# zraorg/ZRA

Measured on AMD Instinct MI355X. Metric: compress + RA-decompress GiB/s, 16 GiB @ 64 KiB frames, 1/2/4/8 MI355X, higher is better.
Workload: dtype u8

## Files before the change

### zra_amd/csrc/zra_encode.hip

```cpp
#include <cstdio>
#include <unistd.h>
#include "zra_host.h"
#include "zra_dev.h"
#include "zra_format.h"
#include "zra_env.h"
#include <algorithm>
#include <cstdlib>
#include <vector>

extern "C" __global__ void zra_mf_kernel(ZraEncArgs a, uint32_t block, uint32_t only, uint32_t onlySlot, uint32_t perWave);
extern "C" __global__ void zra_mf_opt_kernel(ZraEncArgs a, uint32_t block, uint32_t only, uint32_t onlySlot, uint32_t perWave);
extern "C" __global__ void zra_mf_dfast_ls_kernel(ZraEncArgs a, uint32_t block, uint32_t only, uint32_t onlySlot);
extern "C" __global__ void zra_mf_hc_kernel(ZraEncArgs a, uint32_t block, uint32_t only, uint32_t onlySlot);
extern "C" __global__ void zra_mf_fast_kernel(ZraEncArgs a, uint32_t block, uint32_t perWave);
extern "C" __global__ void zra_mf_dfast_kernel(ZraEncArgs a, uint32_t block, uint32_t only, uint32_t onlySlot);
extern "C" __global__ void zra_mf_dfast_fl_kernel(ZraEncArgs a, ZraFlagArgs g, uint32_t block, uint32_t only, uint32_t onlySlot);
extern "C" __global__ void zra_entropy_kernel(ZraEncArgs a, uint32_t block);
extern "C" __global__ void zra_entropy_front_kernel(ZraEncArgs a, uint32_t block);
extern "C" __global__ void zra_entropy_back_kernel(ZraEncArgs a, uint32_t block);
extern "C" __global__ void zra_ent_chain_kernel(ZraEncArgs a);
extern "C" __global__ void zra_ent_chain5_kernel(ZraEncArgs a);

using namespace zra_dev;
using namespace zra_env;
// ... 186 lines not shown
  HIPCHK(hipMemsetAsync(encScan_.p, 0, 64 + 4 * nEntLaunches, stream2_));
  size_t entLaunch = 0;

  ZraEncArgs base{};
  base.in = dIn; base.inSize = inSize; base.frameSize = frameSize; base.checksum = checksum ? 1 : 0;
  base.full = full; base.tail = tail;
  dbgSeqStride_ = seqStride; dbgB_ = (uint32_t)B;
  base.tableStride = tableWords; base.seqStride = seqStride; base.litStride = litStride; base.slotStride = slotStride;
  base.entWorkStride = entWorkStride; base.slotRing = B; base.entSubFrames = B; base.entPrio = 3;

  size_t evNext = 0;
  auto ev = [&]() -> hipEvent_t {
    if (evNext == evPool_.size()) { hipEvent_t e = nullptr; if (hipEventCreate(&e) != hipSuccess) return nullptr; evPool_.push_back(e); }
    return evPool_[evNext++];
  };
  std::vector<std::pair<hipEvent_t, hipEvent_t>> mfSpans, entSpans;
  hipEvent_t entDone[2] = {nullptr, nullptr};
  hipStream_t mfStream2 = nullptr;
  if (nCtx == 2) {
    if (!pipeStreams_[0] && hipStreamCreateWithFlags(&pipeStreams_[0], hipStreamNonBlocking) != hipSuccess) { pipeStreams_[0] = nullptr; (void)hipGetLastError(); }
    mfStream2 = pipeStreams_[0];
  }
  { hipEvent_t e0 = ev(); if (!e0) return zerr(1); HIPCHK(hipEventRecord(e0, stream_)); HIPCHK(hipStreamWaitEvent(stream2_, e0, 0));
    if (mfStream2) HIPCHK(hipStreamWaitEvent(mfStream2, e0, 0)); }

  uint64_t batchIdx = 0;
  for (uint64_t f0 = 0; f0 < nFramesTotal; f0 += B, batchIdx++) {
    const uint32_t nb = (uint32_t)std::min<uint64_t>(B, nFramesTotal - f0);
    const int c = (int)(batchIdx % nCtx);
    EncCtx& x = encCtx_[c];
    ZraEncArgs a = base;
    a.firstFrame = (uint32_t)f0; a.nFrames = nb;
    a.tables = x.tables.as<uint32_t>(); a.seqs = x.seqs.as<uint64_t>(); a.lits = x.lits.as<uint8_t>(); a.slots = x.slots.as<uint8_t>();
    a.state = x.misc.as<ZraEncFrameState>();
    a.blockOut = (ZraEncBlockOut*)(x.misc.as<uint8_t>() + (size_t)B * sizeof(ZraEncFrameState));
    a.contentCk = x.ck.as<uint32_t>();
    a.sizes = x.sizes.as<uint64_t>();
    uint64_t* dOffsets = x.sizes.as<uint64_t>() + B;
    if (checksum)
      hipLaunchKernelGGL(zra_content_ck_kernel, dim3((nb * 4 + 255) / 256), dim3(256), 0, stream2_, dIn, (u64)inSize, frameSize, (u32)f0, nb, a.contentCk);
    const uint64_t firstFrameSize = std::min<uint64_t>(frameSize, inSize - f0 * frameSize);
    const ZraEncParams& P0 = firstFrameSize == frameSize ? full : tail;
    const uint32_t rounds = (uint32_t)((firstFrameSize + P0.blockSize - 1) / P0.blockSize);
    hipStream_t sA = (c == 1 && mfStream2) ? mfStream2 : stream_;
    if (entDone[c]) HIPCHK(hipStreamWaitEvent(sA, entDone[c], 0));
    { static const bool poison = env_set("ZRA_ENC_POISON");
      if (poison) HIPCHK(hipMemsetAsync(x.tables.p, 0xA5, (size_t)nb * tableWords * 4, sA)); }
    for (uint32_t blk = 0; blk < rounds; blk++) {
      hipEvent_t m0 = ev(), m1 = ev(), e1 = ev();
      if (!m0 || !m1 || !e1) return zerr(1);
      HIPCHK(hipEventRecord(m0, sA));
      {
        const bool hasTail = tailSize && f0 + nb == nFramesTotal;
        const uint32_t shL = 1, shS = 2, dupLog = 8;
        a.mfFilter = shL | (shS << 4) | (dupLog << 8);
        const uint32_t hl = std::max(full.hashLog, tail.hashLog), cl = std::max(full.chainLog, tail.chainLog);
        const size_t filterBytes = (8u << dupLog) + (((size_t)1 << hl) >> shL) / 8 + (((size_t)1 << cl) >> shS) / 8 + 64;
        const bool serialAll = std::min<uint64_t>(frameSize, inSize) > (1ull << full.windowLog);
        a.serialAll = serialAll ? 1u : 0u;
        const bool oddTail = !serialAll && hasTail && (tail.strategy == 2) != (full.strategy == 2);
        auto launchLone = [&](uint32_t only, uint32_t slot) {
          if (tail.strategy >= 3 && tail.strategy <= 5) hipLaunchKernelGGL(zra_mf_hc_kernel, dim3(1), dim3(64), 0, sA, a, blk, only, slot);
          else hipLaunchKernelGGL(mfGeneric, dim3(1), dim3(64), 0, sA, a, blk, only, slot, 1u);
        };
        if (full.strategy == 2 && !serialAll) {
          hipLaunchKernelGGL(zra_mf_dfast_kernel, dim3(nb), dim3(64), filterBytes, sA, a, blk, 0xFFFFFFFFu, 0u);
          if (oddTail) launchLone((uint32_t)(nb - 1), (uint32_t)(nb - 1));
        } else {
          const bool hashChain = full.strategy >= 3 && full.strategy <= 5 && !serialAll;
          const uint32_t perWave = hashChain ? 1u : std::min<uint32_t>(8u, std::max<uint32_t>(1u, (nb + (uint32_t)numCUs_ * 32 - 1) / ((uint32_t)numCUs_ * 32)));
          const bool lean = hashChain || full.strategy == 1;
          const uint32_t hcPad = hashChain && full.searchLog >= 5 && tableWords * 4 >= (4ull << 20) ? 5120u : 0u;
          if (hashChain) hipLaunchKernelGGL(zra_mf_hc_kernel, dim3(nb), dim3(64), hcPad, sA, a, blk, 0xFFFFFFFFu, 0u);
          else if (lean) hipLaunchKernelGGL(zra_mf_fast_kernel, dim3((nb + perWave - 1) / perWave), dim3(64), 0, sA, a, blk, perWave);
          else hipLaunchKernelGGL(mfGeneric, dim3((nb + perWave - 1) / perWave), dim3(64), 0, sA, a, blk, 0xFFFFFFFFu, 0u, perWave);
          if (oddTail) hipLaunchKernelGGL(zra_mf_dfast_kernel, dim3(1), dim3(64), filterBytes, sA, a, blk, (uint32_t)(nb - 1), (uint32_t)(nb - 1));
          else if (lean && hasTail && (hashChain ? (tail.strategy < 3 || tail.strategy > 5) : tail.strategy != 1))
            launchLone((uint32_t)(nb - 1), (uint32_t)(nb - 1));
        }
      }
      HIPCHK(hipEventRecord(m1, sA));
      mfSpans.push_back({m0, m1});
      HIPCHK(hipStreamWaitEvent(stream2_, m1, 0));
      hipEvent_t e0 = ev(); if (!e0) return zerr(1);
      HIPCHK(hipEventRecord(e0, stream2_));
      { ZraEncArgs ae = a; ae.entQueue = dEntQueues + entLaunch++; ae.entWork = x.work.as<uint8_t>();
        hipLaunchKernelGGL(zra_entropy_kernel, dim3(std::min<uint32_t>(nb, entGridB)), dim3(256), 0, stream2_, ae, blk); }
      HIPCHK(hipEventRecord(e1, stream2_));
      entSpans.push_back({e0, e1});
      if (blk + 1 < rounds) HIPCHK(hipStreamWaitEvent(sA, e1, 0));
    }
    hipLaunchKernelGGL(zra_scan_sizes_kernel, dim3(1), dim3(64), 0, stream2_, a.sizes, nb, dOffsets, dRunning, (const u32*)nullptr);
    hipLaunchKernelGGL(zra_gather_frames_kernel, dim3(nb), dim3(256), 0, stream2_, a.slots, slotStride, a.sizes, dOffsets, dBody,
                       bodyBase0, dEntries ? dEntries : nullptr, (u32)f0, dSizes, (const u32*)nullptr);
    hipEvent_t done = ev(); if (!done) return zerr(1);
    HIPCHK(hipEventRecord(done, stream2_));
    entDone[c] = done;
    if ((uint64_t)env_i64("ZRA_ENC_FAIL_BATCH", -1) == batchIdx) return zerr(1);
  }
  uint64_t total = 0;
  HIPCHK(hipMemcpyAsync(&total, dRunning, 8, hipMemcpyDeviceToHost, stream2_));
  HIPCHK(hipStreamSynchronize(stream2_));
  HIPCHK(hipStreamSynchronize(stream_));
  if (mfStream2) HIPCHK(hipStreamSynchronize(mfStream2));
  HIPCHK(hipGetLastError());
  double kernelMs = 0;
  kstats_[0] = kstats_[1] = kstats_[2] = kstats_[3] = 0;
  for (auto& sp : mfSpans) { float m = 0; if (hipEventElapsedTime(&m, sp.first, sp.second) == hipSuccess) { kstats_[0] += m; kstats_[1] += 1; kernelMs += m; } }
  for (auto& sp : entSpans) { float m = 0; if (hipEventElapsedTime(&m, sp.first, sp.second) == hipSuccess) { kstats_[2] += m; kstats_[3] += 1; } }
  lastKernelMs_ = kernelMs;
// ... 15 lines not shown
  {
    size_t freeB = 0, totalB = 0;
    if (hipMemGetInfo(&freeB, &totalB) != hipSuccess) freeB = 24ull << 30;
    uint64_t mine = 0; for (auto& x : encCtx_) mine += x.seqs.cap;
    budget = std::min<uint64_t>(64ull << 30, std::max<uint64_t>(8ull << 30, ((uint64_t)freeB + mine) / 3));
  }
  uint64_t SBIG = 0, nSuper = 0, subsPerSuper = 0; int nCtx = 1;
  EncCtx& sh = encCtx_[0];
  static const uint32_t entPerCU = (uint32_t)std::max(1, env_int("ZRA_ENT_WGS", 8));
  const uint32_t entGrid = (uint32_t)std::min<uint64_t>((uint64_t)numCUs_ * entPerCU, nFramesTotal);
  const uint64_t entWorkStride = (9 * seqStride + 255) & ~255ull;
  static const int splitEnv = env_int("ZRA_ENT_SPLIT", 1);
  const bool entSplit = splitEnv >= 2 || (splitEnv == 1 && nFramesTotal >= 256);
  uint64_t slotRing = 0;
  for (;; budget /= 2) {
    SBIG = std::max<uint64_t>(1, std::min<uint64_t>(nFramesTotal, budget / perFrame));
    if (SBIG > SB) SBIG -= SBIG % SB;
    nCtx = nFramesTotal > SBIG ? 2 : 1;
    nSuper = (nFramesTotal + SBIG - 1) / SBIG;
    subsPerSuper = (SBIG + SB - 1) / SB;
    slotRing = std::min<uint64_t>(SB, SBIG);
    const uint64_t workUnits = entSplit ? std::min<uint64_t>(SB, nFramesTotal) : entGrid;
    bool okR = sh.tables.reserve((size_t)nSlots * tableWords * 4) && sh.lits.reserve((size_t)entGrid * litStride) && sh.work.reserve((size_t)workUnits * entWorkStride) &&
               sh.slots.reserve(slotRing * slotStride) && (!entSplit || sh.rec.reserve((size_t)workUnits * sizeof(ZraEntRec)));
    for (int c = 0; c < nCtx && okR; c++) {
      EncCtx& x = encCtx_[c];
      okR = x.seqs.reserve(SBIG * seqStride * 8) && x.misc.reserve(SBIG * (sizeof(ZraEncFrameState) + sizeof(ZraEncBlockOut))) &&
            x.ck.reserve((size_t)SBIG * 4) && x.sizes.reserve((size_t)SBIG * 16);
    }
    if (okR) break;
    if (budget <= (1ull << 30) || SBIG <= SB) return zerr(64);
    (void)hipGetLastError();
  }
  const size_t nCnt = 4 + 8 * (size_t)nSuper + 4 * (size_t)(nSuper * subsPerSuper) + 4;
  const size_t cntCore = (16 + 4 * nCnt + 15) & ~(size_t)15;
  const size_t cntBytes = cntCore + 8 * (size_t)ZRA_TELE_WORDS;
  if (!encScan_.reserve(cntBytes)) return zerr(64);
  uint64_t* dRunning = encScan_.as<uint64_t>();
  uint32_t* dCnt = (uint32_t*)(encScan_.as<uint8_t>() + 16);
  uint32_t* dPerSuper = dCnt + 4;
  uint32_t* dPerSub = dPerSuper + 8 * nSuper;
  HIPCHK(hipMemsetAsync(encScan_.as<uint8_t>(), 0, cntBytes, stream_));
  encCounters_ = dCnt; encCountersBytes_ = 4 * (4 + 8 * (size_t)nSuper + 4 * (size_t)(nSuper * subsPerSuper));

  ZraEncArgs base{};
  base.in = dIn; base.inSize = inSize; base.frameSize = frameSize; base.checksum = checksum ? 1 : 0;
  base.full = full; base.tail = tail;
  dbgSeqStride_ = seqStride; dbgB_ = (uint32_t)SBIG;
  base.tableStride = tableWords; base.seqStride = seqStride; base.litStride = litStride; base.slotStride = slotStride;
  base.mfTele = (uint64_t*)(encScan_.as<uint8_t>() + cntCore);
  base.entWorkStride = entWorkStride;
  base.entPrio = 1;
  base.entSubFrames = SB; base.slotRing = (uint32_t)slotRing; base.readyStamp = 1u;
  const uint32_t shL = 1, shS = 3, dupLog = 8;
  base.mfFilter = shL | (shS << 4) | (dupLog << 8);
  const uint32_t hl = std::max(full.hashLog, tail.hashLog), cl = std::max(full.chainLog, tail.chainLog);
  const size_t filterBytes = (8u << dupLog) + (((size_t)1 << hl) >> shL) / 8 + (((size_t)1 << cl) >> shS) / 8;

  static const int lsEnv = env_int("ZRA_MF_LS", 1);
  const uint32_t lsBytes = (uint32_t)((std::min<uint64_t>(frameSize, inSize) + 64 + 63) & ~63ull);
  const uint32_t lsPerCu = (uint32_t)((160u << 10) / (lsBytes + filterBytes));
  static const int lsMaxEnv = env_int("ZRA_MF_LS_MAX", -1);
  bool useLs = lsEnv != 0 && full.strategy == 2 && lsPerCu >= 1 &&
               nFramesTotal <= (lsMaxEnv >= 0 ? (uint64_t)lsMaxEnv : (uint64_t)lsPerCu * (uint64_t)numCUs_);
  if (useLs && lsAttr_ == 0) {
    const bool okA = hipFuncSetAttribute((const void*)zra_mf_dfast_ls_kernel, hipFuncAttributeMaxDynamicSharedMemorySize, 160 << 10) == hipSuccess;
    if (!okA) (void)hipGetLastError();
    lsAttr_ = okA ? 1 : -1;
  }
  if (lsAttr_ < 0) useLs = false;

  static const int flEnv = env_int("ZRA_MF_FLAGS", 1);
  const bool useFlagsWave = flEnv != 0 && !useLs && full.strategy == 2;
  ZraFlagArgs fw{};
  if (useFlagsWave) {
    fw.flagStride = ((((uint64_t)std::min<uint64_t>(frameSize, inSize) + 511) / 512) * 128 + 255) & ~255ull;
    if (!mfFlags_.reserve((size_t)nSlots * fw.flagStride)) return zerr(64);
    fw.flags = mfFlags_.as<uint8_t>(); fw.ldsWords = (uint32_t)(filterBytes / 4);
    fw.spanBytes = 768;
    static const int epEnv = env_int("ZRA_MF_EPOCH", 4);
    const uint32_t ibMax = 32u - (uint32_t)__builtin_clz((uint32_t)std::max<uint64_t>(2, std::min<uint64_t>(frameSize, inSize)) - 1u);
    fw.epochBits = (uint32_t)std::max(0, std::min(epEnv, (int)(32u - ibMax) - 10));
  }
  const size_t spanLds = fw.spanBytes ? fw.spanBytes + 16 + (fw.spanBytes / 64 + 1) * 16 : 0;

  size_t evNext = 0;
  auto ev = [&]() -> hipEvent_t {
    if (evNext == evPool_.size()) { hipEvent_t e = nullptr; if (hipEventCreate(&e) != hipSuccess) return nullptr; evPool_.push_back(e); }
    return evPool_[evNext++];
  };
  std::vector<std::pair<hipEvent_t, hipEvent_t>> mfSpans, entSpans;
  static const bool traceOn = env_set("ZRA_ENC_TRACE");
  hipEvent_t superDone[2] = {nullptr, nullptr};
  { hipEvent_t e0 = ev(); if (!e0) return zerr(1); HIPCHK(hipEventRecord(e0, stream_)); HIPCHK(hipStreamWaitEvent(stream2_, e0, 0)); }

  for (uint64_t S = 0; S < nSuper; S++) {
    const uint64_t F0 = S * SBIG;
    const uint32_t n = (uint32_t)std::min<uint64_t>(SBIG, nFramesTotal - F0);
    const int c = (int)(S % nCtx);
    EncCtx& x = encCtx_[c];
    ZraEncArgs a = base;
    a.firstFrame = (uint32_t)F0; a.nFrames = n;
    a.tables = sh.tables.as<uint32_t>(); a.lits = sh.lits.as<uint8_t>(); a.slots = sh.slots.as<uint8_t>(); a.entWork = sh.work.as<uint8_t>();
    a.seqs = x.seqs.as<uint64_t>();
    a.state = x.misc.as<ZraEncFrameState>();
    a.blockOut = (ZraEncBlockOut*)(x.misc.as<uint8_t>() + (size_t)SBIG * sizeof(ZraEncFrameState));
    a.contentCk = x.ck.as<uint32_t>();
    a.sizes = x.sizes.as<uint64_t>();
    a.mfQueue = dPerSuper + 8 * S; a.mfStarted = a.mfQueue + 1;
    uint32_t* const entQ = dPerSub + 4 * S * subsPerSuper;
    a.mfDone = entQ + 3 * subsPerSuper;
    if (superDone[c]) HIPCHK(hipStreamWaitEvent(stream_, superDone[c], 0));
    HIPCHK(hipMemsetAsync(a.blockOut, 0, (size_t)n * sizeof(ZraEncBlockOut), stream_));
    hipEvent_t m0 = ev(), m1 = ev();
    if (!m0 || !m1) return zerr(1);
    HIPCHK(hipEventRecord(m0, stream_));
    const uint32_t mfGrid = std::min<uint32_t>(n, nSlots);
    if (useFlagsWave) hipLaunchKernelGGL(zra_mf_dfast_fl_kernel, dim3(mfGrid), dim3(64), filterBytes + spanLds, stream_, a, fw, 0u, 0xFFFFFFFFu, 0u);
    else if (useLs) {
      ZraEncArgs al = a; al.mfFilter |= (lsBytes / 64) << 16;
      hipLaunchKernelGGL(zra_mf_dfast_ls_kernel, dim3(mfGrid), dim3(64), lsBytes + filterBytes, stream_, al, 0u, 0xFFFFFFFFu, 0u);
    } else hipLaunchKernelGGL(zra_mf_dfast_kernel, dim3(mfGrid), dim3(64), filterBytes, stream_, a, 0u, 0xFFFFFFFFu, 0u);
    HIPCHK(hipGetLastError());
    HIPCHK(hipEventRecord(m1, stream_));
    mfSpans.push_back({m0, m1});
    const bool oddTail = tailSize && F0 + n == nFramesTotal && tail.strategy != 2;
    if (oddTail) {
      ZraEncArgs at = a; at.mfQueue = nullptr;
      if (tail.strategy >= 3 && tail.strategy <= 5) hipLaunchKernelGGL(zra_mf_hc_kernel, dim3(1), dim3(64), 0, stream_, at, 0u, (uint32_t)(n - 1), 0u);
      else hipLaunchKernelGGL(mfGeneric, dim3(1), dim3(64), 0, stream_, at, 0u, (uint32_t)(n - 1), 0u, 1u);
    }
    HIPCHK(hipStreamWaitValue32(stream2_, a.mfStarted, mfGrid, hipStreamWaitValueGte, 0xFFFFFFFFu));
    if (checksum)
      hipLaunchKernelGGL(zra_content_ck_kernel, dim3((n * 4 + 255) / 256), dim3(256), 0, stream2_, dIn, (u64)inSize, frameSize, (u32)F0, n, a.contentCk);
    const uint32_t nSub1 = (n + SB - 1) / SB;
    for (uint32_t j = 0; j < nSub1; j++) {
      const uint32_t j0 = j * SB, nbj = std::min<uint32_t>(SB, n - j0);
      const bool hasOdd = oddTail && j == nSub1 - 1;
      HIPCHK(hipStreamWaitValue32(stream2_, a.mfDone + j, nbj - (hasOdd ? 1u : 0u), hipStreamWaitValueGte, 0xFFFFFFFFu));
      if (hasOdd) { hipEvent_t te = ev(); if (!te) return zerr(1); HIPCHK(hipEventRecord(te, stream_)); HIPCHK(hipStreamWaitEvent(stream2_, te, 0)); }
      ZraEncArgs aj = a;
      aj.firstFrame = (uint32_t)(F0 + j0); aj.nFrames = nbj;
      aj.seqs = a.seqs + (size_t)j0 * seqStride; aj.state = a.state + j0; aj.blockOut = a.blockOut + j0;
      aj.contentCk = a.contentCk + j0; aj.sizes = a.sizes + j0;
      aj.entQueue = entQ + j;
      uint64_t* dOffsets = x.sizes.as<uint64_t>() + SBIG + j0;
      hipEvent_t e0 = ev(), e1 = ev(); if (!e0 || !e1) return zerr(1);
      HIPCHK(hipEventRecord(e0, stream2_));
      if (entSplit) {
        aj.entRec = sh.rec.as<ZraEntRec>();
        hipLaunchKernelGGL(zra_entropy_front_kernel, dim3(std::min<uint32_t>(nbj, entGrid)), dim3(256), 0, stream2_, aj, 0u);
        const uint32_t cg = wavesPerCU >= 19 ? 5u : 6u;
        hipLaunchKernelGGL(cg == 5 ? zra_ent_chain5_kernel : zra_ent_chain_kernel, dim3((nbj + cg - 1) / cg), dim3(64), 0, stream2_, aj);
        ZraEncArgs ab = aj; ab.entQueue = entQ + subsPerSuper + j;
        hipLaunchKernelGGL(zra_entropy_back_kernel, dim3(std::min<uint32_t>(nbj, entGrid)), dim3(256), 0, stream2_, ab, 0u);
      } else
        hipLaunchKernelGGL(zra_entropy_kernel, dim3(std::min<uint32_t>(nbj, entGrid)), dim3(256), 0, stream2_, aj, 0u);
      HIPCHK(hipEventRecord(e1, stream2_));
      entSpans.push_back({e0, e1});
      hipLaunchKernelGGL(zra_scan_sizes_kernel, dim3(1), dim3(64), 0, stream2_, aj.sizes, nbj, dOffsets, dRunning, (const u32*)nullptr);
      hipLaunchKernelGGL(zra_gather_frames_kernel, dim3(nbj), dim3(256), 0, stream2_, aj.slots, slotStride, aj.sizes, dOffsets, dBody,
                         bodyBase0, dEntries ? dEntries : nullptr, (u32)(F0 + j0), dSizes, (const u32*)nullptr);
    }
    hipEvent_t done = ev(); if (!done) return zerr(1);
    HIPCHK(hipEventRecord(done, stream2_));
    superDone[c] = done;
  }
  uint64_t total = 0;
  HIPCHK(hipMemcpyAsync(&total, dRunning, 8, hipMemcpyDeviceToHost, stream2_));
  HIPCHK(hipStreamSynchronize(stream2_));
  HIPCHK(hipStreamSynchronize(stream_));
// ... 87 lines not shown
```

### zra_amd/csrc/zra_encode_mf.hip

```cpp
#include "zra_dev.h"
#include "zra_kernels.h"
#include "zra_encode_wave.h"

using namespace zra_dev;
using namespace zra_wave;

#ifdef ZRA_MF_PROFILE
__device__ unsigned long long zra_mf_prof[24];
#define PROF_DECL u64 pt_[20]; for (int k_ = 0; k_ < 20; k_++) pt_[k_] = 0; u64 pl_ = __builtin_amdgcn_s_memtime();
#define PROF(k) { __builtin_amdgcn_s_waitcnt(0); const u64 n_ = __builtin_amdgcn_s_memtime(); pt_[k] += n_ - pl_; pl_ = n_; }
#define PROF_CNT(k) { pt_[k]++; }
#define PROF_END { if (lane == 0) for (int k_ = 0; k_ < 20; k_++) atomicAdd(&zra_mf_prof[k_], pt_[k_]); }
#elif defined(ZRA_MF_MARK)
#define PROF_DECL
#define PROF(k) asm volatile("; ZMARK " #k);
#define PROF_CNT(k)
#define PROF_END
#else
#define PROF_DECL
#define PROF(k)
#define PROF_CNT(k)
#define PROF_END
#endif

// ... 303 lines not shown
          break;
        }
      }
      if (off) {
        const u32 ro = off - 2;
        while (start > anchor && start > ro && src[start - 1] == src[start - ro - 1]) { start--; ml++; }
        o2 = o1; o1 = ro;
      }
    }
    E.put(start - anchor, ml, off ? off + 1 : 1);
    anchor = ip = start + ml;
    while (ip <= ilimit && o2 > 0 && ld32(src + ip) == ld32(src + ip - o2)) {
      const u32 rl = count_eq(src, ip + 4, ip + 4 - o2, be) + 4;
      const u32 t = o2; o2 = o1; o1 = t;
      E.put(0, rl, 1);
      ip += rl; anchor = ip;
    }
  }
  rep[0] = o1 ? o1 : saved; rep[1] = o2 ? o2 : saved;
  return be - anchor;
}



template <u32 MLS, u32 EB = 0>
struct DfHash {
  u32 shL, shS, shT, ib, tagMask;
  u32 epoch;
  __device__ __forceinline__ void init(u32 hlog, u32 clog, u32 ibits, u32 ep = 0) {
    ib = ibits; tagMask = ~((1u << ib) - 1u); shL = 64 - hlog; shS = (MLS == 4 ? 32 : 64) - clog; shT = shL - (32 - ib);
    epoch = ep;
  }
  __device__ __forceinline__ void both(u64 v, u32& bL, u32& bS, u32& tL, u32& tS) const {
    const u64 pl = v * 0xCF1BBCDCB7A56463ULL;
    const u32 p4 = (u32)v * 2654435761u;
    bL = (u32)(pl >> shL);
    if (EB == 0) { tL = (u32)(pl >> shT) << ib; tS = p4 & tagMask; }
    else {
      constexpr u32 keep = ~((1u << EB) - 1u);
      tL = (((u32)(pl >> shT) & keep) | epoch) << ib;
      tS = (((p4 >> ib) & keep) | epoch) << ib;
    }
    if (MLS == 5) bS = (u32)(((v << 24) * 889523592379ULL) >> shS);
    else if (MLS == 6) bS = (u32)(((v << 16) * 227718039650203ULL) >> shS);
    else if (MLS == 7) bS = (u32)(((v << 8) * 58295818150454627ULL) >> shS);
    else bS = p4 >> shS;
  }
};

struct __attribute__((packed, aligned(1))) quad_u { u32 x, y, z, w; };
__device__ __forceinline__ uint4 ld128(const u8* p) { const quad_u q = *(const quad_u*)p; return make_uint4(q.x, q.y, q.z, q.w); }

struct LeanLds {
  u8* dup; u32 dupSlots; u32* bmL; u32* bmS; u32 shL, shS;
  u8* span; u8* spanFlg; u32 spanBytes;
  __device__ __forceinline__ void markL(u32 b) const { const u32 g = b >> shL; atomicOr(&bmL[g >> 5], 1u << (g & 31)); }
  __device__ __forceinline__ void markS(u32 b) const { const u32 g = b >> shS; atomicOr(&bmS[g >> 5], 1u << (g & 31)); }
};

#ifdef ZRA_MF_NT
#define TLD(p) __builtin_nontemporal_load(p)
#define TST(p, v) __builtin_nontemporal_store((u32)(v), p)
#elif defined(ZRA_MF_SC1ST)
#ifdef ZRA_MF_SC1LD
#define TLD(p) __hip_atomic_load((p), __ATOMIC_RELAXED, __HIP_MEMORY_SCOPE_AGENT)
#else
#define TLD(p) (*(p))
#endif
#define TST(p, v) __hip_atomic_store((p), (u32)(v), __ATOMIC_RELAXED, __HIP_MEMORY_SCOPE_AGENT)
#else
#define TLD(p) (*(p))
#define TST(p, v) (*(p) = (v))
#endif
__device__ __forceinline__ u32 df_flags_at(const u8* flg, u32 p) {
  const u8* const w = flg + (size_t)(p >> 6) * 16 + ((p & 63u) >> 3);
  const u32 b = p & 7u;
  return 0x05u | (((w[0] >> b) & 1u) << 1) | (((w[8] >> b) & 1u) << 3);
}
#define ZRA_DF_EPOCH_BITS 4u
template <u32 MLS, bool FLAGS>
__device__ u32 mf_dfast_lean(const ZraEncParams& P, u32* HL, u32* HS, const u8* src, u32 bs, u32 be, u32* rep, u64* seqs, u32* nOut,
                             const LeanLds& W, int lane, u32 ib, const u8* flgIn, u32 epoch = 0) {
  const u8* const flg = FLAGS ? flgIn : nullptr;
  DfHash<MLS, FLAGS ? ZRA_DF_EPOCH_BITS : 0u> H; H.init(P.hashLog, P.chainLog, ib, FLAGS ? rfl(epoch) : 0u);
  const u32 idxMask = ~H.tagMask;
  bs = rfl(bs); be = rfl(be);
  u32 o1 = rfl(rep[0]), o2 = rfl(rep[1]), saved;
  u32 anchor = bs, nseq = 0;
  const u32 ilimit = be >= 8 ? be - 8 : 0;
  u32 ip = mf_prologue(bs, o1, o2, saved);
  u32 sqLo = 0, sqHi = 0;
  u32* const dL = (u32*)W.dup; u32* const dS = dL + W.dupSlots;
  const u32 dmask = W.dupSlots - 1;
  for (u32 i = (u32)lane; i < 2 * W.dupSlots; i += 64) dL[i] = 0;
  u32 dupRound = 0;
  u32* const bmL = W.bmL; u32* const bmS = W.bmS;
  PROF_DECL
  auto emit = [&](u32 ll, u32 ml, u32 offVal) {
    const u64 q = (u64)ll | ((u64)ml << 20) | ((u64)offVal << 40);
    sqLo = wlane(sqLo, (u32)q, nseq & 63); sqHi = wlane(sqHi, (u32)(q >> 32), nseq & 63);
    nseq++;
    if ((nseq & 63) == 0) seqs[nseq - 64 + (u32)lane] = (u64)sqLo | ((u64)sqHi << 32);
  };
  auto insert_slow = [&](u32 pos, bool doL, bool doS) {
    if (lane == 0) {
      const u32 fx = flg ? df_flags_at(flg, pos) : 0x0Fu;
      u32 bl, bs_, tl, ts; H.both(ld64(src + pos), bl, bs_, tl, ts);
      if (doL && (fx & 2)) { TST(HL + bl, (pos + 1) | tl); W.markL(bl); }
      if (doS && (fx & 8)) { TST(HS + bs_, (pos + 1) | ts); W.markS(bs_); }
    }
  };
  const bool useSpan = FLAGS && W.spanBytes != 0;
  u32 sBase = 0, sEnd = 0;
  auto span_fill = [&](u32 at) {
    const u32 mis = (u32)((uintptr_t)(src + at) & 15u);
    const u32 base = rfl(at - min(at, mis));
    const u32 len = min(W.spanBytes, be - base);
    const u32 o = 16u * (u32)lane;
    if (o + 16 <= len) lds_write128(W.span + o, ld128(src + base + o));
    else if (o < len) { for (u32 k = o; k < len; k++) lds_write8(W.span + k, src[base + k]); }
    if (flg) {
      const u32 l2 = (u32)lane, w0 = base >> 6;
      if (l2 <= (W.spanBytes >> 6) && (w0 + l2) * 64u < be) lds_write128(W.spanFlg + 16u * l2, *(const uint4*)(flg + 16u * (size_t)(w0 + l2)));
    }
    __builtin_amdgcn_wave_barrier();
    sBase = base; sEnd = base + len;
  };
  while (ip < ilimit) {
    const u32 wip = ip, run = ip - anchor;
    u32 s = 1, nAct;
    if (run < 256) nAct = min(min(64u, 256u - run), ilimit - ip);
    else { s = (run >> 8) + 1; nAct = min(64u, min((256 * s - run + s - 1) / s, (ilimit - ip + s - 1) / s)); }
    bool active = (u32)lane < nAct;
    const u32 p = wip + (u32)lane * s;
    u64 v8; u32 bflags;
    if (useSpan && s == 1) {
      if (wip < sBase || wip + nAct + 7 > sEnd) span_fill(wip);
      const u32 r = p - sBase;
      v8 = active ? *(const lds_u64u_t*)(W.span + r) : 0;
      bflags = 0x0Fu;
      if (flg && active) {
        const u8* const w = W.spanFlg + ((p >> 6) - (sBase >> 6)) * 16u + ((p & 63u) >> 3);
        const u32 b = p & 7u;
        bflags = 0x05u | (((lds_read8(w) >> b) & 1u) << 1) | (((lds_read8(w + 8) >> b) & 1u) << 3);
      }
    } else {
      v8 = active ? ld64(src + p) : 0;
      bflags = (flg && active) ? df_flags_at(flg, p) : 0x0Fu;
    }
    u32 repFor = o1;
    bool rv = active && o1 > 0 && p + 1 >= o1;
    u32 repVal = rv ? ld32(src + p + 1 - o1) : 0;
    PROF(0) PROF_CNT(12)
    u32 bL, bS, tL, tS; H.both(v8, bL, bS, tL, tS);
    if (nAct > 1) {
      bool pL = active, pS = active;
      u64 mates = 0;
      for (;;) {
        dupRound++;
        const u32 key = (dupRound << 6) | (63u - (u32)lane);
        if (pL) atomicMax(&dL[bL & dmask], key);
        if (pS) atomicMax(&dS[bS & dmask], key);
        __builtin_amdgcn_wave_barrier();
        const u32 wl = pL ? 63u - (lds_read32(&dL[bL & dmask]) & 63u) : (u32)lane;
        const u32 ws = pS ? 63u - (lds_read32(&dS[bS & dmask]) & 63u) : (u32)lane;
        __builtin_amdgcn_wave_barrier();
        const u32 obL = (u32)__shfl((int)bL, (int)wl, 64), obS = (u32)__shfl((int)bS, (int)ws, 64);
        const bool lostL = wl != (u32)lane, lostS = ws != (u32)lane;
        const bool sameL = lostL && obL == bL, sameS = lostS && obS == bS;
        mates |= __ballot(sameL || sameS);
        pL = lostL && !sameL; pS = lostS && !sameS;
        PROF_CNT(17)
        if (!__ballot(pL || pS)) break;
      }
      if (mates) { nAct = (u32)__builtin_ctzll(mates); active = (u32)lane < nAct; }
    }
    PROF(1)
    const u32 gL = bL >> W.shL, gS = bS >> W.shS;
    const u32 wL = gL >> 5, wS = gS >> 5, qL = 1u << (gL & 31), qS = 1u << (gS & 31);
    u32 mL = 0, mS = 0;
    if (active) {
      const bool needL = (bflags & 1) && (bmL[wL] & qL) != 0, needS = (bflags & 4) && (bmS[wS] & qS) != 0;
      const u32 rL = needL ? TLD(HL + bL) : 0u, rS = needS ? TLD(HS + bS) : 0u;
      mL = ((rL & H.tagMask) == tL) ? (rL & idxMask) : 0u;
      mS = ((rS & H.tagMask) == tS) ? (rS & idxMask) : 0u;
    }
    PROF(2)
    u64 LH = __ballot(active && mL > 1);
    u64 SH = __ballot(active && mS > 1);
    const u32 valL = (p + 1) | tL, valS = (p + 1) | tS;
    const u32 v8s = (u32)(v8 >> 8);
    const u64 AM = nAct >= 64 ? ~0ull : (bit64(nAct) - 1);
    u64 RH = __ballot(rv && repVal == v8s);
    u32 repOld = 0, repOldFor = 0xFFFFFFFFu; u64 ROV = 0;
    u64 RV = __ballot(rv);
    PROF(3)
    u32 cur = 0;
    for (;;) {
      if (repFor != o1) {
        rv = active && o1 > 0 && p + 1 >= o1;
        repVal = rv ? ld32(src + p + 1 - o1) : 0; repFor = o1;
        RH = __ballot(rv && repVal == v8s); RV = __ballot(rv);
      }
      const u64 live = AM & (~0ull << cur);
      const u64 hm = (RH | LH | SH) & live;
      if (!hm) {
        if (lane_in(live)) { if (bflags & 2) { TST(HL + bL, valL); atomicOr(&bmL[wL], qL); } if (bflags & 8) { TST(HS + bS, valS); atomicOr(&bmS[wS], qS); } }
        ip = wip + nAct * s; PROF(4)
        break;
      }
      const u32 f = (u32)__builtin_ctzll(hm);
      u64 mkL = live & ((bit64(f) << 1) - 1), mkS = mkL;
      const u32 top = wip + f * s;
      const bool isRep = (RH >> f) & 1, isLong = (LH >> f) & 1;
      ip = top;
      u32 m, known, offVal = 1;
      u32 vneed = 0, mS2 = 0; bool dual = false;
      if (isRep) { ip = top + 1; m = ip - o1; known = 4; }
      else if (isLong) { m = bcast(mL, f) - 1; known = 0; vneed = 8; }
      else if (s == 1 && f + 1 < nAct) {
        mkL |= bit64(f + 1);
        if ((LH >> (f + 1)) & 1) { m = bcast(mL, f + 1) - 1; ip = top + 1; known = 0; vneed = 8; dual = true; mS2 = bcast(mS, f) - 1; }
        else { m = bcast(mS, f) - 1; known = 0; vneed = 4; }
      } else {
        bool hit3; u32 m3;
        {
// ... 536 lines not shown
          const u32 p = blk * 512 + k * 64 + (u32)lane;
          const bool act = p <= lastPos;
          const u32 ci = 8 * k + srcLane;
          const u32 c0l = (u32)__builtin_amdgcn_ds_bpermute((int)(4 * ci), (int)aLo), c0h = (u32)__builtin_amdgcn_ds_bpermute((int)(4 * ci), (int)aHi);
          u32 c1l = (u32)__builtin_amdgcn_ds_bpermute((int)(4 * ((ci + 1) & 63)), (int)aLo), c1h = (u32)__builtin_amdgcn_ds_bpermute((int)(4 * ((ci + 1) & 63)), (int)aHi);
          if (ci == 63) { c1l = (u32)above; c1h = (u32)(above >> 32); }
          const u64 c0 = (u64)c0l | ((u64)c0h << 32), c1 = (u64)c1l | ((u64)c1h << 32);
          const u64 v = sh ? (c0 >> sh) | (c1 << (64 - sh)) : c0;
          const u32 bL = (u32)((v * 0xCF1BBCDCB7A56463ULL) >> (64 - hlog));
          const u32 bS = mls <= 4 ? ((u32)v * 2654435761u) >> (32 - clog) : (u32)(((v << shV) * primeS) >> (64 - clog));
          pLw[h] = act && (bL >> hlogP) == pass; pSw[h] = act && (bS >> clogP) == pass;
          iLw[h] = bL & ((1u << hlogP) - 1); iSw[h] = bS & ((1u << clogP) - 1);
        }
        u32 seenL[2], seenS[2], cL[2], cS[2];
#pragma unroll
        for (int h = 0; h < 2; h++) {
          const u32 iL = iLw[h], iS = iSw[h], sL = iL & 255u, sS = 256u + (iS & 255u);
          const bool pL = pLw[h], pS = pSw[h];
          seenL[h] = pL ? lds_read32(&bmL[iL >> 5]) : 0u; seenS[h] = pS ? lds_read32(&bmS[iS >> 5]) : 0u;
          if (pL) atomicAdd(&cnt[sL >> 2], 1u << (8 * (sL & 3)));
          if (pS) atomicAdd(&cnt[sS >> 2], 1u << (8 * (sS & 3)));
          __builtin_amdgcn_wave_barrier();
          cL[h] = pL ? lds_read32(&cnt[sL >> 2]) : 0u;
          cS[h] = pS ? lds_read32(&cnt[sS >> 2]) : 0u;
          __builtin_amdgcn_wave_barrier();
          if (pL) { atomicSub(&cnt[sL >> 2], 1u << (8 * (sL & 3))); atomicOr(&bmL[iL >> 5], 1u << (iL & 31)); }
          if (pS) { atomicSub(&cnt[sS >> 2], 1u << (8 * (sS & 3))); atomicOr(&bmS[iS >> 5], 1u << (iS & 31)); }
          __builtin_amdgcn_wave_barrier();
        }
#pragma unroll
        for (int h = 0; h < 2; h++) {
          const u32 k = 7 - 2 * kk - h;
          if (blk * 512 + k * 64 > lastPos) continue;
          const u32 iL = iLw[h], iS = iSw[h], sL = iL & 255u, sS = iS & 255u;
          const u64 mL = __ballot(((seenL[h] >> (iL & 31)) & 1u) || ((cL[h] >> (8 * (sL & 3))) & 255u) > 1);
          const u64 mS = __ballot(((seenS[h] >> (iS & 31)) & 1u) || ((cS[h] >> (8 * (sS & 3))) & 255u) > 1);
          if ((u32)lane == 2 * k) outM = mL;
          if ((u32)lane == 2 * k + 1) outM = mS;
        }
      }
      if (lane < 16) *(u64*)(flg + (size_t)blk * 128 + 8 * (u32)lane) = outM | B0.m;
      above = (u64)bcast(aLo, 0) | ((u64)bcast(aHi, 0) << 32);
      B0 = B1;
    }
    __builtin_amdgcn_fence(__ATOMIC_RELEASE, "agent");
    __builtin_amdgcn_fence(__ATOMIC_ACQUIRE, "agent");
  }
}
template <bool FLAGS, bool LSRC = false>
__device__ __forceinline__ void mf_dfast_body(const ZraEncArgs& a, u32 block, u32 only, u32 onlySlot, const ZraFlagArgs* g = nullptr) {
  const int lane = threadIdx.x;
  extern __shared__ u32 dynLds[];
  LeanLds W;
  W.shL = a.mfFilter & 15; W.shS = (a.mfFilter >> 4) & 15; W.dupSlots = 1u << ((a.mfFilter >> 8) & 15);
  u32* const fltLds = LSRC ? dynLds + (a.mfFilter >> 16) * 16 : dynLds;
  W.dup = (u8*)fltLds;
  W.bmL = fltLds + 2 * W.dupSlots;
  W.span = nullptr; W.spanFlg = nullptr; W.spanBytes = 0;
  if (FLAGS && g && g->spanBytes) { W.spanBytes = g->spanBytes; W.span = (u8*)(fltLds + g->ldsWords); W.spanFlg = W.span + g->spanBytes + 16; }
  const bool persistent = a.mfQueue != nullptr;
  const bool tele = persistent && a.mfTele != nullptr;
  u64* const tl = tele ? a.mfTele + ZRA_TELE_HEAD + 4 * (size_t)min(blockIdx.x, ZRA_TELE_WAVES - 1u) : nullptr;
  if (tele && lane == 0) {
    const u32 hw = __builtin_amdgcn_s_getreg((31 << 11) | 4);
    const u32 xcc = __builtin_amdgcn_s_getreg((3 << 11) | 20) & 7u;
    const u64 tc0 = __builtin_readcyclecounter(), tr0 = wall_clock64();
    const u32 key = (xcc << 8) | (((hw >> 13) & 7u) << 5) | (((hw >> 12) & 1u) << 4) | ((hw >> 8) & 15u);
    atomicAdd((unsigned long long*)&a.mfTele[32 + key], 1ull << (16u * ((hw >> 4) & 3u)));
    atomicAdd((unsigned long long*)&a.mfTele[8 + xcc], 1ull);
    atomicMax((unsigned long long*)&a.mfTele[4], ~tr0);
    atomicMax((unsigned long long*)&a.mfTele[6], tr0);
    tl[0] = tc0; tl[1] = tr0; tl[2] = xcc; tl[3] = 0;
  }
  if (persistent && a.mfStarted && lane == 0) atomicAdd(a.mfStarted, 1u);
  const u32 epochBits = (FLAGS && g && persistent) ? min(g->epochBits, ZRA_DF_EPOCH_BITS) : 0u;
  u32 epochCtr = 0;
  for (;;) {
    u32 f = only == 0xFFFFFFFFu ? blockIdx.x : only;
    if (persistent) {
      u32 t = 0;
      if (lane == 0) t = atomicAdd(a.mfQueue, 1u);
      f = rfl(t);
      if (f >= a.nFrames) {
        if (tele && lane == 0) {
          const u64 tc1 = __builtin_readcyclecounter(), tr1 = wall_clock64();
          const u64 tc0 = tl[0], tr0 = tl[1];
          const u32 xcc = (u32)tl[2] & 7u;
          atomicAdd((unsigned long long*)&a.mfTele[0], tc1 - tc0);
          atomicAdd((unsigned long long*)&a.mfTele[1], tr1 - tr0);
          atomicAdd((unsigned long long*)&a.mfTele[2], 1ull);
          atomicMax((unsigned long long*)&a.mfTele[3], tr1 - tr0);
          atomicMax((unsigned long long*)&a.mfTele[5], tr1);
          atomicMax((unsigned long long*)&a.mfTele[7], ~tr1);
          atomicAdd((unsigned long long*)&a.mfTele[16 + xcc], (unsigned long long)tl[3]);
          atomicAdd((unsigned long long*)&a.mfTele[24 + xcc], tr1 - tr0);
        }
        return;
      }
      if (tele && lane == 0) tl[3]++;
    }
#ifdef ZRA_MF_PROFILE
    const u64 kt0_ = __builtin_amdgcn_s_memtime();
#endif
    bool mine = true;
    {
      const u64 fstart = (u64)(a.firstFrame + f) * a.frameSize;
      const ZraEncParams& Pf = (a.inSize - fstart < a.frameSize) ? a.tail : a.full;
      if (Pf.strategy != 2) mine = false;
    }
    MfFrame F;
    bool keepTables = false; u32 epoch = 0;
    if (epochBits && mine) {
      const u64 fstart = (u64)(a.firstFrame + f) * a.frameSize;
      const bool fullFrame = a.inSize - fstart >= a.frameSize;
      if (!fullFrame) epochCtr = 0;
      epoch = epochCtr & ((1u << epochBits) - 1u);
      keepTables = epoch != 0;
      epochCtr = fullFrame ? epochCtr + 1 : 0;
    }
    if (mine && mf_frame_setup(a, block, lane, F, f, persistent ? blockIdx.x : only == 0xFFFFFFFFu ? f : onlySlot, false, keepTables)) {
#ifdef ZRA_MF_PROFILE
      __builtin_amdgcn_s_waitcnt(0);
      if (lane == 0) atomicAdd(&zra_mf_prof[20], __builtin_amdgcn_s_memtime() - kt0_);
#endif
      const u32 wordsL = ((1u << F.P->hashLog) >> W.shL) / 32, wordsS = ((1u << F.P->chainLog) >> W.shS) / 32;
      W.bmS = W.bmL + wordsL;
      u32 rep[3] = {F.st->rep[0], F.st->rep[1], F.st->rep[2]};
      u32 lastLL, nseq = 0;
      const u32 ib = 32 - __builtin_clz(F.fsize - 1);
      const u8* flg = nullptr;
      if (FLAGS && g && g->flags && block == 0 && persistent) {
        u8* const fw = g->flags + (size_t)blockIdx.x * g->flagStride;
        df_later_flags(F.src, F.fsize, F.P->hashLog, F.P->chainLog, F.P->minMatch, fltLds, g->ldsWords, fw, lane);
        flg = fw;
      }
      {
        const u32 fill = block == 0 ? 0u : 0xFFFFFFFFu;
        for (u32 i = lane; i < wordsL + wordsS; i += 64) W.bmL[i] = fill;
        __builtin_amdgcn_fence(__ATOMIC_ACQ_REL, "workgroup");
      }
      const u8* srcP = F.src;
      if (LSRC) {
        u8* const ls = (u8*)dynLds;
        const u32 n16 = F.fsize >> 4;
        for (u32 i = (u32)lane; i < n16; i += 64) *(uint4*)(ls + 16 * i) = ld128(F.src + 16 * i);
        for (u32 i = (n16 << 4) + (u32)lane; i < F.fsize; i += 64) ls[i] = F.src[i];
        ls[F.fsize + (u32)lane] = 0;
        __builtin_amdgcn_fence(__ATOMIC_RELEASE, "workgroup");
        __builtin_amdgcn_wave_barrier();
        __builtin_amdgcn_fence(__ATOMIC_ACQUIRE, "workgroup");
        srcP = ls;
      }
      switch (F.P->minMatch) {
        case 5: lastLL = mf_dfast_lean<5, FLAGS>(*F.P, F.hashT, F.chainT, srcP, F.bs, F.be, rep, F.seqs, &nseq, W, lane, ib, flg, epoch); break;
        case 6: lastLL = mf_dfast_lean<6, FLAGS>(*F.P, F.hashT, F.chainT, srcP, F.bs, F.be, rep, F.seqs, &nseq, W, lane, ib, flg, epoch); break;
        case 7: lastLL = mf_dfast_lean<7, FLAGS>(*F.P, F.hashT, F.chainT, srcP, F.bs, F.be, rep, F.seqs, &nseq, W, lane, ib, flg, epoch); break;
        default: lastLL = mf_dfast_lean<4, FLAGS>(*F.P, F.hashT, F.chainT, srcP, F.bs, F.be, rep, F.seqs, &nseq, W, lane, ib, flg, epoch); break;
      }
      if (lane == 0) {
        F.bo->nbSeq = nseq; F.bo->lastLL = lastLL; F.bo->skip = 0;
        F.bo->rep[0] = rep[0]; F.bo->rep[1] = rep[1]; F.bo->rep[2] = rep[2];
      }
#ifdef ZRA_MF_PROFILE
      __builtin_amdgcn_s_waitcnt(0);
      if (lane == 0) { atomicAdd(&zra_mf_prof[21], __builtin_amdgcn_s_memtime() - kt0_); atomicAdd(&zra_mf_prof[22], 1ull); }
#endif
    }
    if (!persistent) return;
    if (mine) {
      __builtin_amdgcn_fence(__ATOMIC_RELEASE, "agent");
      if (lane == 0) { __hip_atomic_store(&a.blockOut[f].ready, a.readyStamp, __ATOMIC_RELEASE, __HIP_MEMORY_SCOPE_AGENT); if (a.mfDone) atomicAdd(&a.mfDone[f / a.entSubFrames], 1u); }
    }
  }
}

extern "C" __global__ void __launch_bounds__(64)
zra_mf_dfast_kernel(ZraEncArgs a, u32 block, u32 only, u32 onlySlot) { mf_dfast_body<false>(a, block, only, onlySlot); }
extern "C" __global__ void __launch_bounds__(64) __attribute__((amdgpu_waves_per_eu(6)))
zra_mf_dfast_fl_kernel(ZraEncArgs a, ZraFlagArgs g, u32 block, u32 only, u32 onlySlot) { mf_dfast_body<true>(a, block, only, onlySlot, &g); }
extern "C" __global__ void __launch_bounds__(64)
zra_mf_dfast_ls_kernel(ZraEncArgs a, u32 block, u32 only, u32 onlySlot) { mf_dfast_body<false, true>(a, block, only, onlySlot); }

template <bool OPT>
__device__ __forceinline__ void mf_generic(const ZraEncArgs& a, u32 block, u32 only, u32 onlySlot, u32 perWave) {
  const int lane = threadIdx.x;
  const bool all = only == 0xFFFFFFFFu;
// ... 94 lines not shown
```

### zra_amd/csrc/zra_kernels.h

```cpp
#pragma once
#include <stdint.h>
#include <stddef.h>

#ifndef ZRA_HUF_FRAMES
#define ZRA_HUF_FRAMES 2
#endif
#define ZRA_DEC_TBL_LL 0u
#define ZRA_DEC_TBL_ML 512u
#define ZRA_DEC_TBL_OF 1024u
#define ZRA_DEC_TBL_WORDS 1280u
#define ZRA_LDS_TBL_LL 0u
#define ZRA_LDS_TBL_ML 1024u
#define ZRA_LDS_TBL_OF 2048u
#define ZRA_LDS_TBL_WORDS 2304u
#define ZRA_CHAIN_LDS_FRAMES 59u
#define ZRA_CHAIN_RING_WORDS 36u

struct ZraDecFrame {
  uint32_t blkPos, produced, done;
  uint32_t hufValid, hufMaxBits, hufNSym, hufX2;
  uint32_t llValid, mlValid, ofValid, llLog, mlLog, ofLog, ofShare;
  uint32_t rep[3];
  uint32_t fcsLo, fcsHi, fcsHave, hasChecksum, bigWindow;
  uint32_t bpos, bsize, blast;
// ... 138 lines not shown
  uint64_t inSize;
  uint32_t frameSize;
  uint32_t firstFrame;
  uint32_t nFrames;
  uint32_t checksum;
  uint32_t mfFilter;
  uint32_t serialAll;
  ZraEncParams full, tail;
  uint32_t* tables;
  uint64_t tableStride;
  uint64_t* seqs;
  uint64_t seqStride;
  uint8_t* lits;
  uint64_t litStride;
  uint8_t* entWork;
  uint64_t entWorkStride;
  uint8_t* slots;
  uint64_t slotStride;
  ZraEncFrameState* state;
  ZraEncBlockOut* blockOut;
  uint32_t* contentCk;
  uint64_t* sizes;
  uint32_t* mfQueue;
  uint32_t* mfStarted;
  uint32_t* mfDone;
  uint32_t* entQueue;
  uint32_t* entDone;
  uint32_t* scanDone;
  uint32_t* gatherJ;
  uint32_t* gQueue;
  uint32_t* gCopied;
  uint32_t* gatherDone;
  uint32_t* pipeAbort;
  uint64_t* offsets;
  uint64_t* running;
  uint8_t* gBody;
  uint8_t* gEntries;
  uint64_t* gSizesOut;
  uint32_t entSubFrames;
  uint32_t slotRing;
  uint32_t readyStamp;
  uint32_t entPrio;
  uint64_t* mfTele;
  ZraEntRec* entRec;
};
#define ZRA_TELE_CUKEYS 2048u
#define ZRA_TELE_HEAD (32u + ZRA_TELE_CUKEYS)
#define ZRA_TELE_WAVES 8192u
#define ZRA_TELE_ENT (ZRA_TELE_HEAD + 4u * ZRA_TELE_WAVES)
#define ZRA_TELE_WORDS (ZRA_TELE_ENT + 8u + ZRA_TELE_CUKEYS)
struct ZraFlagArgs {
  uint8_t* flags; uint64_t flagStride; uint32_t ldsWords;
  uint32_t spanBytes;
  uint32_t epochBits;
};
```

Before: 20.72.

## Replace LDS atomic dedup of hash buckets with ballot bit-slice comparison

The intra-wave duplicate-bucket detection in the dfast match finder no longer uses an LDS dup table with atomicMax rounds. It now compares bucket indices across lanes bit by bit with ballots and bitop3, stopping early once a conflicting lane is found or all hash bits are covered. Removing the dup table frees LDS, so the flag-sweep kernel gets a larger LDS allocation (sweepWords, rounded to 1280-byte granules) and a wider span buffer. The result is fewer LDS atomics and barriers, in exchange for more ballot/VALU work per step and a different occupancy profile.

Measured after the change: 20.67, median of 4. No clear change (-0.2%).

```diff
diff --git a/zra_amd/csrc/zra_encode.hip b/zra_amd/csrc/zra_encode.hip
--- a/zra_amd/csrc/zra_encode.hip
+++ b/zra_amd/csrc/zra_encode.hip
@@ -262,10 +262,10 @@
       HIPCHK(hipEventRecord(m0, sA));
       {
         const bool hasTail = tailSize && f0 + nb == nFramesTotal;
-        const uint32_t shL = 1, shS = 2, dupLog = 8;
-        a.mfFilter = shL | (shS << 4) | (dupLog << 8);
+        const uint32_t shL = 1, shS = 2;
+        a.mfFilter = shL | (shS << 4);
         const uint32_t hl = std::max(full.hashLog, tail.hashLog), cl = std::max(full.chainLog, tail.chainLog);
-        const size_t filterBytes = (8u << dupLog) + (((size_t)1 << hl) >> shL) / 8 + (((size_t)1 << cl) >> shS) / 8 + 64;
+        const size_t filterBytes = (((size_t)1 << hl) >> shL) / 8 + (((size_t)1 << cl) >> shS) / 8 + 64;
         const bool serialAll = std::min<uint64_t>(frameSize, inSize) > (1ull << full.windowLog);
         a.serialAll = serialAll ? 1u : 0u;
         const bool oddTail = !serialAll && hasTail && (tail.strategy == 2) != (full.strategy == 2);
@@ -387,10 +387,10 @@
   base.entWorkStride = entWorkStride;
   base.entPrio = 1;
   base.entSubFrames = SB; base.slotRing = (uint32_t)slotRing; base.readyStamp = 1u;
-  const uint32_t shL = 1, shS = 3, dupLog = 8;
-  base.mfFilter = shL | (shS << 4) | (dupLog << 8);
+  const uint32_t shL = 1, shS = 3;
+  base.mfFilter = shL | (shS << 4);
   const uint32_t hl = std::max(full.hashLog, tail.hashLog), cl = std::max(full.chainLog, tail.chainLog);
-  const size_t filterBytes = (8u << dupLog) + (((size_t)1 << hl) >> shL) / 8 + (((size_t)1 << cl) >> shS) / 8;
+  const size_t filterBytes = (((size_t)1 << hl) >> shL) / 8 + (((size_t)1 << cl) >> shS) / 8;
 
   static const int lsEnv = env_int("ZRA_MF_LS", 1);
   const uint32_t lsBytes = (uint32_t)((std::min<uint64_t>(frameSize, inSize) + 64 + 63) & ~63ull);
@@ -412,12 +412,17 @@
     fw.flagStride = ((((uint64_t)std::min<uint64_t>(frameSize, inSize) + 511) / 512) * 128 + 255) & ~255ull;
     if (!mfFlags_.reserve((size_t)nSlots * fw.flagStride)) return zerr(64);
     fw.flags = mfFlags_.as<uint8_t>(); fw.ldsWords = (uint32_t)(filterBytes / 4);
-    fw.spanBytes = 768;
+    fw.spanBytes = 1024;
     static const int epEnv = env_int("ZRA_MF_EPOCH", 4);
     const uint32_t ibMax = 32u - (uint32_t)__builtin_clz((uint32_t)std::max<uint64_t>(2, std::min<uint64_t>(frameSize, inSize)) - 1u);
     fw.epochBits = (uint32_t)std::max(0, std::min(epEnv, (int)(32u - ibMax) - 10));
   }
   const size_t spanLds = fw.spanBytes ? fw.spanBytes + 16 + (fw.spanBytes / 64 + 1) * 16 : 0;
+  const size_t sweep2 = 512 + (((size_t)1 << hl) + ((size_t)1 << cl)) / 16;
+  size_t flLds = filterBytes + spanLds;
+  if (sweep2 > flLds && sweep2 <= 6 * 1280) flLds = sweep2;
+  flLds = (flLds + 1279) / 1280 * 1280;
+  fw.sweepWords = (uint32_t)(flLds / 4);
 
   size_t evNext = 0;
   auto ev = [&]() -> hipEvent_t {
@@ -451,7 +456,7 @@
     if (!m0 || !m1) return zerr(1);
     HIPCHK(hipEventRecord(m0, stream_));
     const uint32_t mfGrid = std::min<uint32_t>(n, nSlots);
-    if (useFlagsWave) hipLaunchKernelGGL(zra_mf_dfast_fl_kernel, dim3(mfGrid), dim3(64), filterBytes + spanLds, stream_, a, fw, 0u, 0xFFFFFFFFu, 0u);
+    if (useFlagsWave) hipLaunchKernelGGL(zra_mf_dfast_fl_kernel, dim3(mfGrid), dim3(64), flLds, stream_, a, fw, 0u, 0xFFFFFFFFu, 0u);
     else if (useLs) {
       ZraEncArgs al = a; al.mfFilter |= (lsBytes / 64) << 16;
       hipLaunchKernelGGL(zra_mf_dfast_ls_kernel, dim3(mfGrid), dim3(64), lsBytes + filterBytes, stream_, al, 0u, 0xFFFFFFFFu, 0u);
diff --git a/zra_amd/csrc/zra_encode_mf.hip b/zra_amd/csrc/zra_encode_mf.hip
--- a/zra_amd/csrc/zra_encode_mf.hip
+++ b/zra_amd/csrc/zra_encode_mf.hip
@@ -379,7 +379,7 @@
 __device__ __forceinline__ uint4 ld128(const u8* p) { const quad_u q = *(const quad_u*)p; return make_uint4(q.x, q.y, q.z, q.w); }
 
 struct LeanLds {
-  u8* dup; u32 dupSlots; u32* bmL; u32* bmS; u32 shL, shS;
+  u32* bmL; u32* bmS; u32 shL, shS;
   u8* span; u8* spanFlg; u32 spanBytes;
   __device__ __forceinline__ void markL(u32 b) const { const u32 g = b >> shL; atomicOr(&bmL[g >> 5], 1u << (g & 31)); }
   __device__ __forceinline__ void markS(u32 b) const { const u32 g = b >> shS; atomicOr(&bmS[g >> 5], 1u << (g & 31)); }
@@ -417,10 +417,6 @@
   const u32 ilimit = be >= 8 ? be - 8 : 0;
   u32 ip = mf_prologue(bs, o1, o2, saved);
   u32 sqLo = 0, sqHi = 0;
-  u32* const dL = (u32*)W.dup; u32* const dS = dL + W.dupSlots;
-  const u32 dmask = W.dupSlots - 1;
-  for (u32 i = (u32)lane; i < 2 * W.dupSlots; i += 64) dL[i] = 0;
-  u32 dupRound = 0;
   u32* const bmL = W.bmL; u32* const bmS = W.bmS;
   PROF_DECL
   auto emit = [&](u32 ll, u32 ml, u32 offVal) {
@@ -481,24 +477,24 @@
     PROF(0) PROF_CNT(12)
     u32 bL, bS, tL, tS; H.both(v8, bL, bS, tL, tS);
     if (nAct > 1) {
-      bool pL = active, pS = active;
-      u64 mates = 0;
-      for (;;) {
-        dupRound++;
-        const u32 key = (dupRound << 6) | (63u - (u32)lane);
-        if (pL) atomicMax(&dL[bL & dmask], key);
-        if (pS) atomicMax(&dS[bS & dmask], key);
-        __builtin_amdgcn_wave_barrier();
-        const u32 wl = pL ? 63u - (lds_read32(&dL[bL & dmask]) & 63u) : (u32)lane;
-        const u32 ws = pS ? 63u - (lds_read32(&dS[bS & dmask]) & 63u) : (u32)lane;
-        __builtin_amdgcn_wave_barrier();
-        const u32 obL = (u32)__shfl((int)bL, (int)wl, 64), obS = (u32)__shfl((int)bS, (int)ws, 64);
-        const bool lostL = wl != (u32)lane, lostS = ws != (u32)lane;
-        const bool sameL = lostL && obL == bL, sameS = lostS && obS == bS;
-        mates |= __ballot(sameL || sameS);
-        pL = lostL && !sameL; pS = lostS && !sameS;
+      const u64 lt = bit64((u32)lane) - 1;
+      const u32 nbits = rfl(max(P.hashLog, P.chainLog));
+      u32 dLl = 0, dLh = 0, dSl = 0, dSh = 0;
+      u64 mates;
+      auto slice = [&](u32 k) {
+        const u32 xL = (u32)__builtin_amdgcn_sbfe((int)bL, k, 1u), xS = (u32)__builtin_amdgcn_sbfe((int)bS, k, 1u);
+        const u64 qL = __ballot((int)xL < 0), qS = __ballot((int)xS < 0);
+        dLl = __builtin_amdgcn_bitop3_b32(xL, dLl, (u32)qL, 0xde); dLh = __builtin_amdgcn_bitop3_b32(xL, dLh, (u32)(qL >> 32), 0xde);
+        dSl = __builtin_amdgcn_bitop3_b32(xS, dSl, (u32)qS, 0xde); dSh = __builtin_amdgcn_bitop3_b32(xS, dSh, (u32)(qS >> 32), 0xde);
+      };
+#pragma unroll
+      for (u32 k = 0; k < 12; k++) slice(k);
+      for (u32 k = 12;; k += 4) {
+        mates = __ballot(active && ((~(dLl & dSl) & (u32)lt) | (~(dLh & dSh) & (u32)(lt >> 32))) != 0);
         PROF_CNT(17)
-        if (!__ballot(pL || pS)) break;
+        if (!mates || k >= nbits) break;
+#pragma unroll
+        for (u32 j = 0; j < 4; j++) slice(k + j);
       }
       if (mates) { nAct = (u32)__builtin_ctzll(mates); active = (u32)lane < nAct; }
     }
@@ -1141,10 +1137,9 @@
   const int lane = threadIdx.x;
   extern __shared__ u32 dynLds[];
   LeanLds W;
-  W.shL = a.mfFilter & 15; W.shS = (a.mfFilter >> 4) & 15; W.dupSlots = 1u << ((a.mfFilter >> 8) & 15);
+  W.shL = a.mfFilter & 15; W.shS = (a.mfFilter >> 4) & 15;
   u32* const fltLds = LSRC ? dynLds + (a.mfFilter >> 16) * 16 : dynLds;
-  W.dup = (u8*)fltLds;
-  W.bmL = fltLds + 2 * W.dupSlots;
+  W.bmL = fltLds;
   W.span = nullptr; W.spanFlg = nullptr; W.spanBytes = 0;
   if (FLAGS && g && g->spanBytes) { W.spanBytes = g->spanBytes; W.span = (u8*)(fltLds + g->ldsWords); W.spanFlg = W.span + g->spanBytes + 16; }
   const bool persistent = a.mfQueue != nullptr;
@@ -1220,7 +1215,7 @@
       const u8* flg = nullptr;
       if (FLAGS && g && g->flags && block == 0 && persistent) {
         u8* const fw = g->flags + (size_t)blockIdx.x * g->flagStride;
-        df_later_flags(F.src, F.fsize, F.P->hashLog, F.P->chainLog, F.P->minMatch, fltLds, g->ldsWords, fw, lane);
+        df_later_flags(F.src, F.fsize, F.P->hashLog, F.P->chainLog, F.P->minMatch, fltLds, g->sweepWords, fw, lane);
         flg = fw;
       }
       {
diff --git a/zra_amd/csrc/zra_kernels.h b/zra_amd/csrc/zra_kernels.h
--- a/zra_amd/csrc/zra_kernels.h
+++ b/zra_amd/csrc/zra_kernels.h
@@ -214,5 +214,6 @@
 struct ZraFlagArgs {
   uint8_t* flags; uint64_t flagStride; uint32_t ldsWords;
   uint32_t spanBytes;
+  uint32_t sweepWords;
   uint32_t epochBits;
 };
```
